# ltinphan/convex-mpc-unitree-go2

Measured on AMD Instinct MI355X. Metric: batched QP solves/sec (N=16, 4-leg friction cone) at 1/2/4/8 MI355X, higher is better.
Workload: dtype f32

## Files before the change

convex-mpc-unitree-go2_amd/csrc/cmpc_condense.h:

```cpp
#pragma once
#include "cmpc_instance.h"

namespace cmpc {

template <int NC>
__device__ __forceinline__ void condense_finish(Smem<NC>& s, f4 (&M)[Cfg<NC>::NTL], int n,
                                                float shift) {
  using C = Cfg<NC>;
  const int lane = opaque_lane();
  const int g = lane >> 4, c = lane & 15;
#pragma unroll
  for (int I = 0; I < C::TT; ++I) {
    const float rs = s.Rt[16 * I + c] + shift;
#pragma unroll
    for (int J = 0; J <= I; ++J) {
      if (J != I && 16 * I + 16 <= n) continue;
      f4 v = M[tile_index(I, J)];
      const int col = 16 * J + c;
#pragma unroll
      for (int q = 0; q < 4; ++q) {
        const int row = 16 * I + 4 * g + q;
        const bool pad = row >= n || col >= n;
        if (J == I) {
          const bool dg = 4 * g + q == c;
// ... 195 lines not shown
        if (kI[J] >= t) continue;
        f4 d = {0.f, 0.f, 0.f, 0.f};
#pragma unroll
        for (int q = 0; q < 3; ++q) d = mfma4(aA[q], Gd[J][q], d);
        Gd[J] = d;
      }
    }
    const int p0 = s.off[t], p1 = s.off[t + 1];
#pragma unroll
    for (int J = 0; J < C::TT; ++J) {
      if (16 * J + 15 < p0 || 16 * J >= p1) continue;
      const int p = 16 * J + c;
      if (p >= p0 && p < p1) {
        const float* bp = &s.Bt[p * kBS + 3 * g];
        Gd[J] = f4{bp[0], bp[1], bp[2], 0.f};
      }
    }
#pragma unroll
    for (int I = 0; I < C::TT; ++I) {
      if (16 * I + 15 < p0 || 16 * I >= p1) continue;
      const int p = 16 * I + c;
      float a[3] = {0.f, 0.f, 0.f};
      if (p >= p0 && p < p1) {
#pragma unroll
        for (int q = 0; q < 3; ++q) a[q] = Cs[p * 12 + 3 * g + q];
      }
#pragma unroll
      for (int J = 0; J <= I; ++J) {
        f4 acc = M[tile_index(I, J)];
#pragma unroll
        for (int q = 0; q < 3; ++q) acc = mfma4(a[q], Gd[J][q], acc);
        M[tile_index(I, J)] = acc;
      }
    }
  }
  mirror_diagonals<NC>(s, M, n, N);
  condense_finish<NC>(s, M, n, shift);
}

__device__ __forceinline__ void step_sums(int k, int N, float& S0, float& S1, float& S2) {
  S0 = (float)(N - k);
  S1 = (float)((N * (N - 1) - k * (k - 1)) >> 1);
  S2 = (float)(((N - 1) * N * (2 * N - 1) - (k - 1) * k * (2 * k - 1)) / 6);
}

template <int NC>
__device__ __forceinline__ void condense_tiles_nil(Smem<NC>& s, const KParams& P,
                                                   f4 (&M)[Cfg<NC>::NTL], int n, float shift) {
  using C = Cfg<NC>;
  const int lane = opaque_lane();
  const int g = lane >> 4, c = lane & 15;
  const int N = P.N;
  n = uniform(n);
  const int TA = (n + 15) >> 4;
  float* Vs = s.G;
  {
    const int sc = lane_state(c);
    float aN[3];
#pragma unroll
    for (int q = 0; q < 3; ++q) {
      const int r = 3 * g + q;
      aN[q] = (sc >= 0) ? s.A[sc * 12 + r] - ((sc == r) ? 1.f : 0.f) : 0.f;
    }
    WSYNC();
#pragma unroll
    for (int J = 0; J < C::TT; ++J) {
      if (J >= TA) continue;
      const int p = 16 * J + c;
      float bt[3];
#pragma unroll
      for (int q = 0; q < 3; ++q) bt[q] = (p < n) ? s.Bt[p * kBS + 3 * g + q] : 0.f;
      f4 d = {0.f, 0.f, 0.f, 0.f};
#pragma unroll
      for (int q = 0; q < 3; ++q) d = mfma4(aN[q], bt[q], d);
#pragma unroll
      for (int q = 0; q < 3; ++q) Vs[p * 12 + 3 * g + q] = d[q];
    }
  }
  WSYNC();
  float q2[3];
#pragma unroll
  for (int q = 0; q < 3; ++q) q2[q] = s.Q2[3 * g + q];
  float uc[C::TT][3], vc[C::TT][3];
#pragma unroll
  for (int J = 0; J < C::TT; ++J) {
    const int p = 16 * J + c;
    const bool ok = J < TA && p < n;
    const float kf = ok ? (float)s.par[p] : 0.f;
#pragma unroll
    for (int q = 0; q < 3; ++q) {
      vc[J][q] = ok ? Vs[p * 12 + 3 * g + q] : 0.f;
      uc[J][q] = ok ? fmaf(-kf, vc[J][q], s.Bt[p * kBS + 3 * g + q]) : 0.f;
    }
  }
#pragma unroll
  for (int I = 0; I < C::TT; ++I) {
    if (I >= TA) {
#pragma unroll
      for (int J = 0; J <= I; ++J) M[tile_index(I, J)] = f4{0.f, 0.f, 0.f, 0.f};
      continue;
    }
    float x[3], y[3];
    {
      const int p = 16 * I + c;
      const bool ok = p < n;
      const int k = ok ? s.par[p] : 0;
      float S0, S1, S2;
      step_sums(k, N, S0, S1, S2);
#pragma unroll
      for (int q = 0; q < 3; ++q) {
        const float v = vc[I][q];
        const float u = uc[I][q];
        x[q] = q2[q] * fmaf(S0, u, S1 * v);
        y[q] = q2[q] * fmaf(S1, u, S2 * v);
      }
    }
#pragma unroll
    for (int J = 0; J <= I; ++J) {
      float u[3], v[3];
#pragma unroll
      for (int q = 0; q < 3; ++q) {
        u[q] = uc[J][q];
        v[q] = vc[J][q];
      }
      f4 acc = {0.f, 0.f, 0.f, 0.f};
#pragma unroll
      for (int q = 0; q < 3; ++q) acc = mfma4(x[q], u[q], acc);
#pragma unroll
      for (int q = 0; q < 3; ++q) acc = mfma4(y[q], v[q], acc);
      M[tile_index(I, J)] = acc;
    }
  }
  mirror_diagonals<NC>(s, M, n, N);
  condense_finish<NC>(s, M, n, shift);
}

template <class SM>
__device__ __forceinline__ bool nilpotent_step(SM& s) {
  const int lane = opaque_lane();
  WSYNC();
  bool nz = false;
#pragma unroll
  for (int e0 = 0; e0 < 144; e0 += 64) {
    const int e = e0 + lane;
    if (e < 144) {
      const int i = e / 12, j = e % 12;
      float acc = 0.f;
#pragma unroll
      for (int k = 0; k < 12; ++k) {
        const float nik = s.A[i * 12 + k] - ((i == k) ? 1.f : 0.f);
        const float nkj = s.A[k * 12 + j] - ((k == j) ? 1.f : 0.f);
        acc = fmaf(nik, nkj, acc);
      }
      nz |= acc != 0.f;
    }
  }
  return __any(nz) == 0;
}

template <int NC>
__device__ __forceinline__ void condense_tiles(Smem<NC>& s, const KParams& P,
                                               f4 (&M)[Cfg<NC>::NTL], int n, float shift,
                                               bool nil = false) {
  if (nil) {
    condense_tiles_nil<NC>(s, P, M, n, shift);
    return;
  }
  if constexpr (NC <= 128) {
    if (P.latency_mode) {
      condense_tiles_bc<NC>(s, P, M, n, shift);
      return;
    }
  }
  condense_tiles_fwd<NC>(s, P, M, n, shift);
}

}
```

convex-mpc-unitree-go2_amd/csrc/cmpc_factor.h:

```cpp
#pragma once
#include "cmpc_instance.h"

namespace cmpc {

__device__ __forceinline__ float diag_element(const f4& d, int c) {
  const int qs = c & 3;
  return qs == 0 ? d[0] : qs == 1 ? d[1] : qs == 2 ? d[2] : d[3];
}

constexpr int kSweepPipeMaxNC = 128;
template <int NC, int K, class SM>
__device__ __forceinline__ void sweep_publish(SM& s, const f4 (&M)[Cfg<NC>::NTL], int sub,
                                              int g, int c) {
  using C = Cfg<NC>;
  const int c0 = 4 * sub;
  const int pc = c - c0;
  const bool colw = pc >= 0 && pc < 4;
  if (colw) {
#pragma unroll
    for (int I = K; I < C::TT; ++I) {
      f4 m = M[tile_index(I, K)];
      if (I == K) {
#pragma unroll
        for (int q = 0; q < 4; ++q) m[q] -= (4 * g + q == c) ? 1.f : 0.f;
// ... 128 lines not shown
        sweep_mfma<NC, -1, false, K>(M, a, b, TA);
        sweep_diagfix<NC, K>(M, sub, g, c);
      }
    }
    sweep_block_plain<NC, K + 1>(s, M, ng, TA, g, c);
  }
}

template <int NC, class SM>
__device__ __forceinline__ void ldl_tiles(SM& s, f4 (&M)[Cfg<NC>::NTL], int n) {
  using C = Cfg<NC>;
  const int lane = opaque_lane();
  const int g = lane >> 4, c = lane & 15;
  n = uniform(n);
  const int TA = (n + 15) >> 4;
#pragma unroll
  for (int I = 0; I < C::TT; ++I) {
    const float dg = diag_element(M[tile_index(I, I)], c);
    const int p = 16 * I + c;
    const float r = (p < n && dg > 0.f) ? rsqrtf(dg) : 1.f;
    if ((c >> 2) == g) s.ds[p] = r;
  }
  WSYNC();
#pragma unroll
  for (int I = 0; I < C::TT; ++I) {
    const f4 ri = *reinterpret_cast<const f4*>(&s.ds[16 * I + 4 * g]);
#pragma unroll
    for (int J = 0; J <= I; ++J) {
      const float cj = s.ds[16 * J + c];
      f4& m = M[tile_index(I, J)];
#pragma unroll
      for (int q = 0; q < 4; ++q) m[q] *= ri[q] * cj;
    }
  }
  const int ng = (n + 3) >> 2;
  if constexpr (NC <= kSweepPipeMaxNC) {
    if (ng > 0) {
      float a[C::TT], b[C::TT];
      sweep_publish<NC, 0>(s, M, 0, g, c);
      sweep_operands<NC, 0>(s, 0, g, c, a, b);
      sweep_block<NC, 0>(s, M, ng, TA, g, c, a, b);
    }
  } else {
    sweep_block_plain<NC, 0>(s, M, ng, TA, g, c);
  }
  float* rinvs = s.pan;
  WSYNC();
  const int lane_r = opaque_lane();
  const int g_r = lane_r >> 4, c_r = lane_r & 15;
#pragma unroll
  for (int p0 = 0; p0 < NC; p0 += 64) {
    const int p = p0 + lane_r;
    if (p < NC) rinvs[p] = 1.f / s.ds[p];
  }
  WSYNC();
#pragma unroll
  for (int I = 0; I < C::TT; ++I) {
    const f4 ri = *reinterpret_cast<const f4*>(&s.ds[16 * I + 4 * g_r]);
    const f4 rinv = *reinterpret_cast<const f4*>(&rinvs[16 * I + 4 * g_r]);
#pragma unroll
    for (int J = 0; J <= I; ++J) {
      const float cj = s.ds[16 * J + c_r];
      f4& m = M[tile_index(I, J)];
#pragma unroll
      for (int q = 0; q < 4; ++q) m[q] *= (J < I) ? rinv[q] * cj : -(ri[q] * cj);
    }
  }
}

template <int NC, class SM>
__device__ __forceinline__ void ldl_apply(SM& s, const f4 (&M)[Cfg<NC>::NTL], int n,
                                          const float* in, float* out) {
  using C = Cfg<NC>;
  CMPC_T0(t_sv);
  const int lane = opaque_lane();
  const int g = lane >> 4, c = lane & 15;
  n = uniform(n);
  const int TA = (n + 15) >> 4;
  WSYNC();
  float zc[C::TT];
  float bc[C::TT];
#pragma unroll
  for (int I = 0; I < C::TT; ++I) bc[I] = 0.f;
#pragma unroll
  for (int I = 0; I < C::TT; ++I) {
    if (I >= TA) {
      if (c == 0) *reinterpret_cast<f4*>(&out[16 * I + 4 * g]) = f4{0.f, 0.f, 0.f, 0.f};
      continue;
    }
    f4 zr = *reinterpret_cast<const f4*>(&in[16 * I + 4 * g]);
    if (I > 0) {
      f2 r01 = {0.f, 0.f}, r23 = {0.f, 0.f};
#pragma unroll
      for (int J = 0; J < I; ++J) {
        const f4 m = M[tile_index(I, J)];
        const f2 zj = {zc[J], zc[J]};
        r01 = __builtin_elementwise_fma(f2{m[0], m[1]}, zj, r01);
        r23 = __builtin_elementwise_fma(f2{m[2], m[3]}, zj, r23);
      }
      zr[0] -= row16_sum(r01[0]);
      zr[1] -= row16_sum(r01[1]);
      zr[2] -= row16_sum(r23[0]);
      zr[3] -= row16_sum(r23[1]);
    }
#pragma unroll
    for (int q = 0; q < 4; ++q) zr[q] = (16 * I + 4 * g + q < n) ? zr[q] : 0.f;
    if (c == 0) *reinterpret_cast<f4*>(&out[16 * I + 4 * g]) = zr;
    WSYNC();
    zc[I] = out[16 * I + c];
  }
#pragma unroll
  for (int I = C::TT - 1; I >= 0; --I) {
    if (I >= TA) continue;
    const f4 zr = *reinterpret_cast<const f4*>(&out[16 * I + 4 * g]);
    const f4 d = M[tile_index(I, I)];
    const float t =
        fmaf(d[3], zr[3], fmaf(d[2], zr[2], fmaf(d[1], zr[1], fmaf(d[0], zr[0], -bc[I]))));
    float xc = col4_sum(t);
    xc = (16 * I + c < n) ? xc : 0.f;
    WSYNC();
    if (g == 0) out[16 * I + c] = xc;
    if (I == 0) break;
    WSYNC();
    const f4 xr = *reinterpret_cast<const f4*>(&out[16 * I + 4 * g]);
#pragma unroll
    for (int J = 0; J < I; ++J) {
      const f4 m = M[tile_index(I, J)];
      bc[J] = fmaf(m[3], xr[3], fmaf(m[2], xr[2], fmaf(m[1], xr[1], fmaf(m[0], xr[0], bc[J]))));
    }
  }
  WSYNC();
  CMPC_ACC(3, t_sv);
  CMPC_CNT(13, 1);
}

template <int NC>
__device__ __forceinline__ void park_store(float* __restrict__ park, const f4 (&M)[Cfg<NC>::NTL]) {
  const int lane = opaque_lane();
#pragma unroll
  for (int t = 0; t < Cfg<NC>::NTL; ++t)
    *reinterpret_cast<f4*>(&park[t * 256 + lane * 4]) = M[t];
}

template <int NC>
__device__ __forceinline__ void park_load(const float* __restrict__ park, f4 (&M)[Cfg<NC>::NTL]) {
  const int lane = opaque_lane();
  asm volatile("s_waitcnt vmcnt(0)\n\tbuffer_inv sc1" ::: "memory");
#pragma unroll
  for (int t = 0; t < Cfg<NC>::NTL; ++t)
    M[t] = *reinterpret_cast<const f4*>(&park[t * 256 + lane * 4]);
}

}
```

convex-mpc-unitree-go2_amd/csrc/cmpc_gradient.h:

```cpp
#pragma once
#include "cmpc_condense.h"

namespace cmpc {

template <class SM>
__device__ __forceinline__ void gradient_powers(SM& s, f4 (&pw)[4], f4 (&tw)[4]) {
  const int lane = opaque_lane();
  const int g = lane >> 4, c = lane & 15;
  const int sc = lane_state(c);
  f4 Pd = {0.f, 0.f, 0.f, 0.f}, Td = {0.f, 0.f, 0.f, 0.f};
#pragma unroll
  for (int q = 0; q < 3; ++q) {
    const int r = 3 * g + q;
    Pd[q] = (sc >= 0) ? s.A[r * 12 + sc] : 0.f;
    Td[q] = (sc >= 0) ? s.A[sc * 12 + r] : 0.f;
  }
  pw[0] = Pd;
  tw[0] = Td;
  if (uniform(s.nil)) {
#pragma unroll
    for (int l = 1; l < 4; ++l) {
#pragma unroll
      for (int q = 0; q < 4; ++q) {
        const float dl = (sc == 3 * g + q && q < 3) ? 1.f : 0.f;
        pw[l][q] = fmaf((float)(1 << l), Pd[q] - dl, dl);
        tw[l][q] = fmaf((float)(1 << l), Td[q] - dl, dl);
      }
    }
    return;
  }
#pragma unroll
  for (int l = 1; l < 4; ++l) {
    f4 pn = {0.f, 0.f, 0.f, 0.f}, tn = {0.f, 0.f, 0.f, 0.f};
#pragma unroll
    for (int q = 0; q < 3; ++q) {
      pn = mfma4(tw[l - 1][q], pw[l - 1][q], pn);
      tn = mfma4(pw[l - 1][q], tw[l - 1][q], tn);
    }
    pw[l] = pn;
    tw[l] = tn;
  }
}

template <int NC, int W>
constexpr bool kGradLat = W > 1 || (Cfg<NC>::WPE == 1 && NC <= 160);
template <int NC, bool LAT = false, bool PREC = false>
__device__ __forceinline__ void gradient(Smem<NC>& s, const KParams& P, int n, const float* vin,
                                         float* gout, const f4* pwc = nullptr,
                                         const f4* twc = nullptr) {
  CMPC_T0(t_gr);
  const int lane = opaque_lane();
  const int g = lane >> 4, c = lane & 15;
  const int N = P.N;
  n = uniform(n);
  WSYNC();
  f4 Et = {0.f, 0.f, 0.f, 0.f};
  double Eh[3] = {0.0, 0.0, 0.0};
  if constexpr (LAT) {
    const int cc = (c < N) ? c : 0;
    const int p0 = s.off[cc], p1 = s.off[cc + 1];
    float dt[3], bv[12][3], vv[12];
#pragma unroll
    for (int q = 0; q < 3; ++q) dt[q] = s.Dt[12 * cc + 3 * g + q];
#pragma unroll
    for (int i = 0; i < 12; ++i) {
      const int p = min(p0 + i, NC - 1);
#pragma unroll
      for (int q = 0; q < 3; ++q) bv[i][q] = s.Bt[p * kBS + 3 * g + q];
      vv[i] = vin[p];
    }
    if constexpr (PREC) {
#pragma unroll
      for (int q = 0; q < 3; ++q) Eh[q] = (double)dt[q];
#pragma unroll
      for (int i = 0; i < 12; ++i) {
        const bool ok = p0 + i < p1;
#pragma unroll
        for (int q = 0; q < 3; ++q) Eh[q] = ok ? fma((double)bv[i][q], (double)vv[i], Eh[q]) : Eh[q];
      }
#pragma unroll
      for (int q = 0; q < 3; ++q) {
        if (c >= N) Eh[q] = 0.0;
        Et[q] = (float)Eh[q];
      }
    } else {
#pragma unroll
      for (int q = 0; q < 3; ++q) Et[q] = dt[q];
#pragma unroll
      for (int i = 0; i < 12; ++i) {
        const bool ok = p0 + i < p1;
#pragma unroll
        for (int q = 0; q < 3; ++q) Et[q] = ok ? fmaf(bv[i][q], vv[i], Et[q]) : Et[q];
      }
      if (c >= N) Et = f4{0.f, 0.f, 0.f, 0.f};
    }
  } else if (c < N) {
    const int p1 = s.off[c + 1];
    if constexpr (PREC) {
#pragma unroll
      for (int q = 0; q < 3; ++q) Eh[q] = (double)s.Dt[12 * c + 3 * g + q];
      for (int p = s.off[c]; p < p1; ++p) {
        const float* bt = &s.Bt[p * kBS + 3 * g];
        const double vp = (double)vin[p];
#pragma unroll
        for (int q = 0; q < 3; ++q) Eh[q] = fma((double)bt[q], vp, Eh[q]);
      }
#pragma unroll
      for (int q = 0; q < 3; ++q) Et[q] = (float)Eh[q];
    } else {
#pragma unroll
      for (int q = 0; q < 3; ++q) Et[q] = s.Dt[12 * c + 3 * g + q];
      for (int p = s.off[c]; p < p1; ++p) {
        const float* bt = &s.Bt[p * kBS + 3 * g];
        const float vp = vin[p];
#pragma unroll
        for (int q = 0; q < 3; ++q) Et[q] = fmaf(bt[q], vp, Et[q]);
      }
    }
  }
  if (uniform(s.nil)) {
    const int sc = lane_state(c);
    float aN[3], aNt[3];
#pragma unroll
    for (int q = 0; q < 3; ++q) {
      const int r = 3 * g + q;
      const float dl = (sc == r) ? 1.f : 0.f;
      aN[q] = (sc >= 0) ? s.A[sc * 12 + r] - dl : 0.f;
      aNt[q] = (sc >= 0) ? s.A[r * 12 + sc] - dl : 0.f;
    }
    if constexpr (PREC) {
      double u64[3];
#pragma unroll
      for (int q = 0; q < 3; ++q) {
        double x = Eh[q], y;
        row_scan2<false>(x, y);
        Eh[q] = x;
        u64[q] = y;
      }
      const int sr = ((c >> 2) < 3) ? 3 * (c & 3) + (c >> 2) : -1;
      d4 acc = {Eh[0], Eh[1], Eh[2], 0.0};
#pragma unroll
      for (int q = 0; q < 3; ++q) {
        const int r = 3 * g + q;
        const double a = (sr >= 0) ? (double)(s.A[sr * 12 + r] - ((sr == r) ? 1.f : 0.f)) : 0.0;
        acc = __builtin_amdgcn_mfma_f64_16x16x4f64(a, u64[q], acc, 0, 0, 0);
      }
#pragma unroll
      for (int q = 0; q < 3; ++q) Et[q] = (float)acc[q];
    } else {
    f4 u = {0.f, 0.f, 0.f, 0.f};
#pragma unroll
    for (int q = 0; q < 3; ++q) {
      float x = Et[q], y;
      row_scan2<false>(x, y);
      Et[q] = x;
      u[q] = y;
    }
#pragma unroll
    for (int q = 0; q < 3; ++q) Et = mfma4(aN[q], u[q], Et);
    }
    if (c < N) {
#pragma unroll
      for (int q = 0; q < 3; ++q) s.E[12 * c + 3 * g + q] = Et[q];
    }
    f4 Lt = {0.f, 0.f, 0.f, 0.f}, v = {0.f, 0.f, 0.f, 0.f};
#pragma unroll
    for (int q = 0; q < 3; ++q) {
      float x = (c < N) ? s.Q2[3 * g + q] * Et[q] : 0.f, y;
      row_scan2<true>(x, y);
      Lt[q] = x;
      v[q] = y;
    }
#pragma unroll
    for (int q = 0; q < 3; ++q) Lt = mfma4(aNt[q], v[q], Lt);
    if (c < N) {
#pragma unroll
      for (int q = 0; q < 3; ++q) s.L[12 * c + 3 * g + q] = Lt[q];
    }
  } else {
  f4 pw[4], tw[4];
  if (pwc != nullptr) {
#pragma unroll
    for (int l = 0; l < 4; ++l) {
      pw[l] = pwc[l];
      tw[l] = twc[l];
    }
  } else {
    gradient_powers(s, pw, tw);
  }
#pragma unroll
  for (int l = 0; l < 4; ++l) {
    if ((1 << l) >= N) break;
    f4 sh = {0.f, 0.f, 0.f, 0.f};
#pragma unroll
    for (int q = 0; q < 3; ++q) sh[q] = row_shift_pow2<false>(Et[q], l);
#pragma unroll
    for (int q = 0; q < 3; ++q) Et = mfma4(tw[l][q], sh[q], Et);
  }
  if (c < N) {
#pragma unroll
    for (int q = 0; q < 3; ++q) s.E[12 * c + 3 * g + q] = Et[q];
  }
  f4 Lt = {0.f, 0.f, 0.f, 0.f};
#pragma unroll
  for (int q = 0; q < 3; ++q) Lt[q] = (c < N) ? s.Q2[3 * g + q] * Et[q] : 0.f;
#pragma unroll
  for (int l = 0; l < 4; ++l) {
    if ((1 << l) >= N) break;
    f4 sh = {0.f, 0.f, 0.f, 0.f};
#pragma unroll
    for (int q = 0; q < 3; ++q) sh[q] = row_shift_pow2<true>(Lt[q], l);
#pragma unroll
    for (int q = 0; q < 3; ++q) Lt = mfma4(pw[l][q], sh[q], Lt);
  }
  if (c < N) {
#pragma unroll
    for (int q = 0; q < 3; ++q) s.L[12 * c + 3 * g + q] = Lt[q];
  }
  }
  WSYNC();
  for (int p = lane; p < n; p += 64) {
    const int k = s.par[p];
    const f4* l = reinterpret_cast<const f4*>(&s.L[12 * k]);
    f2 a2 = {s.Rt[p] * vin[p], 0.f};
    const f4* bt = reinterpret_cast<const f4*>(&s.Bt[p * kBS]);
#pragma unroll
    for (int j = 0; j < 3; ++j) {
      const f4 lv = l[j], bv = bt[j];
      a2 = __builtin_elementwise_fma(f2{bv[0], bv[1]}, f2{lv[0], lv[1]}, a2);
      a2 = __builtin_elementwise_fma(f2{bv[2], bv[3]}, f2{lv[2], lv[3]}, a2);
    }
    gout[p] = a2[0] + a2[1];
  }
  WSYNC();
  CMPC_ACC(2, t_gr);
  CMPC_CNT(12, 1);
}

}
```

convex-mpc-unitree-go2_amd/csrc/cmpc_solve.h:

```cpp
#pragma once
#include "cmpc_team.hip"

#include "cmpc_condense.h"
#include "cmpc_factor.h"
#include "cmpc_gradient.h"
#include "cmpc_polish.h"

namespace cmpc {

template <int NC>
__device__ __forceinline__ int session_start(Smem<NC>& s, const KParams& P, int ntri, int nfail,
                                             int& ntried, bool& seen) {
  const int l = opaque_lane();
  WSYNC();
  uint8_t c = 0;
  if (l < ntri) {
    c = (uint8_t)s.code[l];
    s.tpat[0][l] = c;
  }
  ntried = 1;
  seen = false;
#pragma unroll
  for (int k = 0; k < kFailMem; ++k) {
    if (k >= nfail) break;
    const bool diff = (l < ntri) && (s.fpat[k][l] != c);
    seen |= (__any(diff) == 0);
  }
  if (seen) return 0;
  return (nfail >= 2) ? min(P.polish_repairs, kLateRepairs) : P.polish_repairs;
}

template <int NC>
__device__ __forceinline__ bool tried_before(Smem<NC>& s, int ntri, int ntried) {
  const int l = opaque_lane();
  WSYNC();
  const uint8_t c = (l < ntri) ? (uint8_t)s.tcnt[l] : 0;
  bool hit = false;
  for (int k = 0; k < ntried; ++k) {
    const bool diff = (l < ntri) && (s.tpat[k][l] != c);
    hit |= (__any(diff) == 0);
  }
  return hit;
}


template <int NC>
constexpr bool kRhoLow = (NC == 128) || (kRhoLowHeavy && NC > 128);

struct Instance {
  int64_t b;
  int N, NP;
  Terrain T;
  bool weights_ok;
  float r2_min;
  const float* Bg;
  const float* xrb;
  int ntri, n;
  bool nil;
  const f4* pwc;
  const f4* twc;
};

struct Ctl {
  int status = -2, iters = 0;
  bool polished = false;
  float rp = 0.f, rd = 0.f, np_ = 0.f, nd = 0.f;
  float rho = 0.f;
  bool rho_low = false;
  int stable = 0;
  bool refactor = false;
  bool in_polish = false;
  int nact = 0;
  float shift = 0.f;
  int it = 0;
  int repairs_left = 0;
  int nadd = 0;
  bool from_cand = false;
  bool parked = false;
  int nfail = 0;
  int ntried = 0;
  bool seen_start = false;
  int last_pol = 0;
  bool fail_rho_done = false;
  bool warm_session = false;
};

__device__ __forceinline__ void set_rho(Ctl& c, const KParams& P, float rho, bool low) {
  c.rho = rho;
  c.rho_low = low;
  c.shift = uniformf(P.sigma + c.rho);
  c.refactor = true;
}

template <int NC>
__device__ __forceinline__ void stage_instance(Smem<NC>& s, const KParams& P, const Inputs& in,
                                               Instance& I, int lane) {
  const int64_t b = I.b;
  const int N = I.N, NP = I.NP;
  const Terrain T = I.T;
  bool weights_ok = true;
  float r2_min = P.r2_min;
  const float* Ab = in.Ad + b * 144;
  const float* Bg = in.Bd + b * (int64_t)N * 144;
  const float* gdb = in.gd + b * 12;
  const float* x0b = in.x0 + b * 12;
  const float* xrb = in.xref + b * (int64_t)N * 12;
  const uint8_t* ctb = in.contact + b * (int64_t)4 * N;

  WSYNC();
  const uint8_t ctv = (lane < 4 * N) ? ctb[(lane & 3) * N + (lane >> 2)] : (uint8_t)0;
  float bw[36];
  if (lane < 4 * N) {
    const float* src = Bg + lane * 36;
#pragma unroll
    for (int i = 0; i < 36; ++i) bw[i] = src[i];
  } else {
#pragma unroll
    for (int i = 0; i < 36; ++i) bw[i] = 0.f;
  }
  {
    float av[3], rv[4];
#pragma unroll
    for (int i = 0; i < 3; ++i) {
      const int e = lane + 64 * i;
      av[i] = (e < 144) ? Ab[e] : 0.f;
    }
#pragma unroll
    for (int i = 0; i < 4; ++i) {
      const int e = lane + 64 * i;
      rv[i] = (e < 12) ? x0b[e] : (e < 12 * (N + 1)) ? xrb[e - 12] : 0.f;
    }
    const float gv = (lane < 12) ? gdb[lane] : 0.f;
    if (in.Q || in.R) {
      const float q = (in.Q && lane < 12) ? in.Q[b * 12 + lane] : 0.f;
      const float r = (in.R && lane < 12) ? in.R[b * 12 + lane] : 1.f;
      weights_ok = __any(!(q >= 0.f && isfinite(q) && r > 0.f && isfinite(r))) == 0;
      if (lane < 12) {
        if (in.Q) s.Q2[lane] = weights_ok ? 2.f * q : 0.f;
        if (in.R) s.R2[lane] = weights_ok ? 2.f * r : 2.f;
      }
      if (in.R)
        r2_min = weights_ok ? uniformf(-wave_max((lane < 12) ? -2.f * r : -INFINITY)) : 2.f;
    }
#pragma unroll
    for (int i = 0; i < 3; ++i) {
      const int e = lane + 64 * i;
      if (e < 144) s.A[e] = av[i];
    }
#pragma unroll
    for (int i = 0; i < 4; ++i) s.G[lane + 64 * i] = rv[i];
    if (lane < 12) s.G[256 + lane] = gv;
  }
  const bool stc = lane < 4 * N && terrain_valid(T) && weights_ok && ctv != 0;
  const int pos = wave_excl_scan4(stc ? 1 : 0);
  const int ntri = wave_total4(stc ? 1 : 0);
  if (stc) s.tri[pos] = lane;
  if (lane < 4 * N) s.tri_of[lane] = stc ? pos : -1;
  WSYNC();
  {
    for (int o = lane; o < NP; o += 64) {
      const int k = o / 12, r = o % 12;
      const float* rk = &s.G[12 * k];
      float acc = s.G[256 + r] - rk[12 + r];
#pragma unroll
      for (int j = 0; j < 12; ++j) acc = fmaf(s.A[r * 12 + j], rk[j], acc);
      s.D[o] = acc;
    }
    build_admm_basis<NC>(s, P, Bg, ntri, &bw, __ballot(stc));
  }
  const bool nil = nilpotent_step(s);
  if (lane == 0) s.nil = nil ? 1 : 0;
// ... 281 lines not shown
    if (__any((nc & oc) != oc) == 0 && c.nadd + nf <= dd_max(NC)) {
      CMPC_T0(t_dd);
      dd = face_downdate<NC>(s, I.T, M, c.nact, ntri, c.nadd);
      TRACEF(I.b, "it %d downdate nf %d -> %d nadd %d\n", c.it, nf, (int)dd, c.nadd);
      CMPC_ACC(28, t_dd);
      CMPC_CNT(29, 1);
      CMPC_CNT(30, nf);
    }
  }
  if (lane < ntri) {
    s.code[lane] = s.tcnt[lane];
    if (c.ntried < kTryMem) s.tpat[c.ntried][lane] = (uint8_t)s.tcnt[lane];
  }
  if (c.ntried < kTryMem) ++c.ntried;
  if (dd) return;
  refactor_faces<NC>(s, P, I, c, s.z);
}

template <int NC>
__device__ __forceinline__ void warm_restart(Smem<NC>& s, const KParams& P, const Instance& I,
                                             Ctl& c) {
  c.warm_session = false;
  build_admm_basis<NC>(s, P, I.Bg, I.ntri);
  {
    const int l = opaque_lane();
    for (int p = l; p < I.n; p += 64) { s.x[p] = 0.f; s.z[p] = 0.f; s.y[p] = 0.f; }
    s.pcode[l] = -1;
  }
  WSYNC();
  c.in_polish = false;
  c.nact = I.n;
  c.nadd = 0;
  set_rho(c, P, kRhoLow<NC> ? 0.5f * P.rho0 : P.rho0, kRhoLow<NC>);
  c.stable = 0;
  c.last_pol = 0;
  c.ntried = 0;
  c.seen_start = false;
  c.parked = false;
}

template <int NC, int W>
__device__ __forceinline__ void session_failed(Smem<NC>& s, const KParams& P, const Instance& I,
                                               Ctl& c, f4 (&M)[TeamCfg<NC, W>::SLOTS],
                                               float* __restrict__ park, TeamSmem<NC, W>* ts,
                                               int* seq, Diag& diag, int lane) {
  c.warm_session = false;
  TRACEF(I.b, "it %d SESSION-FAIL nfail %d seen %d parked %d rho_low %d fail_rho_done %d nadd %d\n",
         c.it, c.nfail, (int)c.seen_start, (int)c.parked, (int)c.rho_low, (int)c.fail_rho_done,
         c.nadd);
  diag.session_failed();
  if (!c.seen_start) {
    const int l = opaque_lane();
    if (l < I.ntri) s.fpat[c.nfail % kFailMem][l] = s.tpat[0][l];
    ++c.nfail;
  }
  build_admm_basis<NC>(s, P, I.Bg, I.ntri);
  c.in_polish = false;
  c.nact = I.n;
  if (c.nfail == 1 && !c.seen_start && kFailRho != 1.f && !c.fail_rho_done) {
    c.fail_rho_done = true;
    set_rho(c, P, uniformf(kFailRho * P.rho0), false);
    return;
  }
  if (c.rho_low) {
    set_rho(c, P, uniformf(P.rho0), false);
    return;
  }
  c.shift = uniformf(P.sigma + c.rho);
  if (c.parked) {
    restore_tiles<NC, W>(park, ts, seq, M);
  } else {
    c.refactor = true;
  }
}

template <int NC, int W>
__device__ __forceinline__ bool admm_iteration(Smem<NC>& s, const KParams& P, const Instance& I,
                                               Ctl& c, const f4 (&M)[TeamCfg<NC, W>::SLOTS],
                                               TeamSmem<NC, W>* ts, int* seq, int lane) {
  const int n = I.n, ntri = I.ntri, it = c.it;
  const Terrain T = I.T;
  const float alpha = P.alpha;
  float rho = c.rho;
  gradient<NC, kGradLat<NC, W>>(s, P, n, s.x, s.g, I.pwc, I.twc);
  {
    const int l = opaque_lane();
    if (l < ntri) {
#pragma unroll
      for (int a = 0; a < 3; ++a) {
        const int p = 3 * l + a;
        s.r[p] = rho * (s.z[p] - s.x[p]) - s.g[p] - s.y[p];
      }
    }
  }
  apply_factors<NC, W>(s, ts, seq, M, n, s.r, s.dl);
  CMPC_T0(t_rest);
  const bool last = (it == P.max_iter);
  const bool adapt = P.adaptive_interval > 0 && (it % P.adaptive_interval) == 0;
  const float inv_rho = 1.f / rho;
  float lrp = 0.f, lrd = 0.f, lnp = 0.f, lnd = 0.f;
  bool changed = false;
  {
    const int l = opaque_lane();
    if (l < ntri) {
      float w[3], xr[3], xs[3];
#pragma unroll
      for (int a = 0; a < 3; ++a) {
        const int p = 3 * l + a;
        const float x = s.x[p], z = s.z[p];
        const float xt = x + s.dl[p];
        xr[a] = alpha * xt + (1.f - alpha) * z;
        xs[a] = alpha * xt + (1.f - alpha) * x;
        w[a] = xr[a] + s.y[p] * inv_rho;
      }
      float pv[3];
      const int code = project(w[0], w[1], w[2], T.mu, T.fz_min, pv[0], pv[1], pv[2]);
#pragma unroll
      for (int a = 0; a < 3; ++a) {
        const int p = 3 * l + a;
        const float zn = pv[a];
        const float yn = s.y[p] + rho * (xr[a] - zn);
        s.x[p] = xs[a];
        s.z[p] = zn;
        s.y[p] = yn;
        const float gp = s.g[p];
        lrp = fmaxf(lrp, fabsf(xs[a] - zn));
        lrd = fmaxf(lrd, fabsf(gp + yn));
        lnp = fmaxf(lnp, fmaxf(fabsf(xs[a]), fabsf(zn)));
        lnd = fmaxf(lnd, fmaxf(fabsf(gp), fabsf(yn)));
      }
      changed = code != s.pcode[l];
      s.pcode[l] = code;
      s.code[l] = code;
    }
  }
  if (trace_on(I.b)) {
    const float trp = wave_max(lrp), trd = wave_max(lrd);
    TRACEF(I.b, "it %d rho %g rp %g rd %g stable %d\n", it, rho, trp, trd, c.stable);
  }
  c.stable = (__any(changed) != 0) ? 0 : c.stable + 1;
  bool do_pol = false;
  const int pstable = P.polish_stable;
  const int backoff = pstable << min(c.nfail, kBackoffCap);
  int need = pstable;
  for (int f = 0; f < min(c.nfail, kBackoffCap); ++f) need *= kStableGrow;
  if (c.stable >= need && !last && it - c.last_pol >= backoff &&
      (P.check_every == 1 || it % P.check_every == 0)) {
    do_pol = true;
    c.last_pol = it;
    c.stable = -backoff;
  }
  if (adapt || last) {
    c.rp = wave_max(lrp); c.rd = wave_max(lrd); c.np_ = wave_max(lnp); c.nd = wave_max(lnd);
  }
  if (adapt && !last) {
    float q = rho * sqrtf((c.rp / fmaxf(c.np_, 1e-30f)) / (c.rd / fmaxf(c.nd, 1e-30f) + 1e-30f));
    q = fminf(fmaxf(q, 1e-6f), 1e6f);
    if (q > 5.f * rho || q < 0.2f * rho) set_rho(c, P, uniformf(q), false);
  }
  CMPC_ACC(7, t_rest);
  return do_pol;
}

template <int NC, int W>
__device__ __forceinline__ void start_session(Smem<NC>& s, const KParams& P, const Instance& I,
                                              Ctl& c, const f4 (&M)[TeamCfg<NC, W>::SLOTS],
                                              float* __restrict__ park, TeamSmem<NC, W>* ts,
                                              int* seq, Diag& diag, int lane) {
  CMPC_CNT(9, 1);
  diag.polish_attempt();
  CMPC_T0(t_ps);
  const bool pending = c.refactor;
  c.parked = !c.refactor && !c.rho_low && c.nfail > 0;
  if (c.parked) park_tiles<NC, W>(park, ts, seq, M);
  enter_polish<NC>(s, P, I, c);
  TRACEF(I.b, "it %d SESSION nfail %d parked %d rho %g refactor_pending %d seen %d repairs %d nact %d\n",
         c.it, c.nfail, (int)c.parked, c.rho, (int)pending, (int)c.seen_start, c.repairs_left,
         c.nact);
  CMPC_ACC(14, t_ps);
}

template <int NC>
__device__ __forceinline__ int force_triple(const Smem<NC>& s, int o, int& a) {
  const int k = o / 12, l = (o % 12) / 3;
  a = o % 3;
  return s.tri_of[4 * k + l];
}

template <int NC>
__device__ __forceinline__ bool write_w(Smem<NC>& s, const Instance& I, float* wb, bool polished,
                                        int lane) {
  const int NP = I.NP;
  const float* uf = polished ? s.x : s.z;
  int bad = 0;
  for (int o = lane; o < NP; o += 64) {
    const float xv = s.E[o] + I.xrb[o];
    int a;
    const int t = force_triple(s, o, a);
    const float uv = (t >= 0) ? uf[3 * t + a] : 0.f;
    bad |= !(isfinite(xv) && isfinite(uv));
    wb[o] = xv;
    wb[NP + o] = uv;
  }
  return __any(bad) == 0;
}

template <int NC, int W>
__device__ __forceinline__ void write_y(Smem<NC>& s, const KParams& P, const Instance& I,
                                        float* yb, bool polished, int lane) {
  const int NP = I.NP;
  if (polished && I.n > 0) {
    build_admm_basis<NC>(s, P, I.Bg, I.ntri);
    gradient<NC, kGradLat<NC, W>>(s, P, I.n, s.x, s.g, I.pwc, I.twc);
  }
  const float* yf = polished ? s.g : s.y;
  const float sg = polished ? -1.f : 1.f;
  for (int o = lane; o < NP; o += 64) {
    int a;
    const int t = force_triple(s, o, a);
    yb[o] = (t >= 0) ? sg * yf[3 * t + a] : 0.f;
  }
}

template <int NC>
__device__ __forceinline__ void write_lam(Smem<NC>& s, const Instance& I, float* lb, bool polished,
                                          int lane) {
  const int N = I.N, NP = I.NP;
  const Terrain T = I.T;
  if (!I.weights_ok) {
    for (int o = lane; o < 52 * N; o += 64) lb[o] = 0.f;
// ... 150 lines not shown
```

convex-mpc-unitree-go2_amd/csrc/cmpc_wave_prims.h:

```cpp
#pragma once
#include <hip/hip_runtime.h>
#include <stdint.h>

namespace cmpc {

typedef float f4 __attribute__((ext_vector_type(4)));
typedef float f2 __attribute__((ext_vector_type(2)));

__device__ __forceinline__ float readlane_f(float v, int lane) {
  return __int_as_float(__builtin_amdgcn_readlane(__float_as_int(v), lane));
}

template <int CTRL>
__device__ __forceinline__ float dpp(float v) {
  return __int_as_float(__builtin_amdgcn_mov_dpp(__float_as_int(v), CTRL, 0xF, 0xF, true));
}

__device__ __forceinline__ int uniform(int v) { return __builtin_amdgcn_readfirstlane(v); }
__device__ __forceinline__ float uniformf(float v) {
  return __builtin_bit_cast(float, __builtin_amdgcn_readfirstlane(__builtin_bit_cast(int, v)));
}

__device__ __forceinline__ void pair32(float v, float& a, float& b) {
  const auto r = __builtin_amdgcn_permlane32_swap(__float_as_int(v), __float_as_int(v), false, false);
  a = __int_as_float(r[0]);
  b = __int_as_float(r[1]);
}
__device__ __forceinline__ void pair16(float v, float& a, float& b) {
  const auto r = __builtin_amdgcn_permlane16_swap(__float_as_int(v), __float_as_int(v), false, false);
  a = __int_as_float(r[0]);
  b = __int_as_float(r[1]);
}

__device__ __forceinline__ float wave_max(float v) {
  v = fmaxf(v, dpp<0xB1>(v));
  v = fmaxf(v, dpp<0x4E>(v));
  v = fmaxf(v, dpp<0x141>(v));
  v = fmaxf(v, dpp<0x140>(v));
  float a, b;
  pair32(v, a, b);
  v = fmaxf(a, b);
  pair16(v, a, b);
  return fmaxf(a, b);
}

__device__ __forceinline__ int wave_excl_scan4(int v) {
  const unsigned long long b0 = __ballot(v & 1), b1 = __ballot(v & 2);
  const int c0 = __builtin_amdgcn_mbcnt_hi((unsigned)(b0 >> 32), __builtin_amdgcn_mbcnt_lo((unsigned)b0, 0));
  const int c1 = __builtin_amdgcn_mbcnt_hi((unsigned)(b1 >> 32), __builtin_amdgcn_mbcnt_lo((unsigned)b1, 0));
  return c0 + 2 * c1;
}
__device__ __forceinline__ int wave_total4(int v) {
  return __popcll(__ballot(v & 1)) + 2 * __popcll(__ballot(v & 2));
}

__device__ __forceinline__ f4 mfma4(float a, float b, f4 c) {
  return __builtin_amdgcn_mfma_f32_16x16x4f32(a, b, c, 0, 0, 0);
}

typedef double d4 __attribute__((ext_vector_type(4)));

template <int CTRL>
__device__ __forceinline__ double dpp64(double v) {
  const long long b = __double_as_longlong(v);
  const int lo = __builtin_amdgcn_mov_dpp((int)(unsigned)(b & 0xffffffffll), CTRL, 0xF, 0xF, true);
  const int hi = __builtin_amdgcn_mov_dpp((int)(b >> 32), CTRL, 0xF, 0xF, true);
  return __longlong_as_double(((long long)hi << 32) | (long long)(unsigned)lo);
}

__device__ __forceinline__ float row16_sum(float v) {
  v += dpp<0xB1>(v);
  v += dpp<0x4E>(v);
  v += dpp<0x141>(v);
  v += dpp<0x140>(v);
  return v;
}

template <bool SHL, int D>
__device__ __forceinline__ float row_shift(float v) { return dpp<(SHL ? 0x100 : 0x110) + D>(v); }
template <bool SHL, int D>
__device__ __forceinline__ double row_shift(double v) { return dpp64<(SHL ? 0x100 : 0x110) + D>(v); }
template <bool SHL>
__device__ __forceinline__ float row_shift_pow2(float v, int l) {
  switch (l) {
    case 0: return row_shift<SHL, 1>(v);
    case 1: return row_shift<SHL, 2>(v);
    case 2: return row_shift<SHL, 4>(v);
    default: return row_shift<SHL, 8>(v);
  }
}
template <bool SHL, class T>
__device__ __forceinline__ void row_scan2(T& x, T& y) {
  x += row_shift<SHL, 1>(x);
  x += row_shift<SHL, 2>(x);
  x += row_shift<SHL, 4>(x);
  x += row_shift<SHL, 8>(x);
  y = row_shift<SHL, 1>(x);
  y += row_shift<SHL, 1>(y);
  y += row_shift<SHL, 2>(y);
  y += row_shift<SHL, 4>(y);
  y += row_shift<SHL, 8>(y);
}

__device__ __forceinline__ float col4_sum(float v) {
  float a, b;
  pair32(v, a, b);
  pair16(a + b, a, b);
  return a + b;
}

__device__ __forceinline__ float wave_sum(float v) { return col4_sum(row16_sum(v)); }

__device__ __forceinline__ int opaque_lane() {
  int l = threadIdx.x & 63;
  asm volatile("" : "+v"(l));
  return l;
}

#define WSYNC() asm volatile("" ::: "memory")

#include "cmpc_diag.h"
#ifdef CMPC_STAMPS
__device__ unsigned long long g_stamps[32];
#define CMPC_FENCE()                                            \
  do {                                                          \
    __builtin_amdgcn_sched_barrier(0);                          \
    asm volatile("s_waitcnt vmcnt(0) lgkmcnt(0)" ::: "memory"); \
    __builtin_amdgcn_sched_barrier(0);                          \
  } while (0)
#define CMPC_T0(name) \
  CMPC_FENCE();       \
  const unsigned long long name = __builtin_amdgcn_s_memtime()
#define CMPC_ACC(ph, t0)                                                              \
  do {                                                                                \
    CMPC_FENCE();                                                                     \
    const unsigned long long _t1 = __builtin_amdgcn_s_memtime();                      \
    if (threadIdx.x == 0) s.st[ph] += _t1 - (t0);                                     \
  } while (0)
#define CMPC_CNT(ph, v) \
  do { if (threadIdx.x == 0) s.st[ph] += (unsigned long long)(v); } while (0)
#else
#define CMPC_T0(name) (void)0
#define CMPC_ACC(ph, t0) (void)0
#define CMPC_CNT(ph, v) (void)0
#endif

}
```

Baseline: 9.474 million.

## Fuse ADMM rhs into gradient epilogue and pipeline triangular solve reductions

Bundles several micro-optimizations: the ADMM right-hand side is now computed inside the gradient close loop through an epilogue lambda, which removes a separate pass over shared memory. The forward LDL substitution is software-pipelined, accumulating the next tile's off-diagonal products early, and its four row reductions are interleaved. Padding masks are precomputed per lane and the backward loads are prefetched. DPP scans are interleaved across the three components, parent indices are cached in registers, and integer modulo is replaced by counters and a cached 1/rho. These cut dependency chains and ALU work per ADMM iteration, at the cost of more register pressure and some added code complexity.

```diff
diff --git a/convex-mpc-unitree-go2_amd/csrc/cmpc_condense.h b/convex-mpc-unitree-go2_amd/csrc/cmpc_condense.h
--- a/convex-mpc-unitree-go2_amd/csrc/cmpc_condense.h
+++ b/convex-mpc-unitree-go2_amd/csrc/cmpc_condense.h
@@ -301,11 +301,13 @@
 #pragma unroll
   for (int q = 0; q < 3; ++q) q2[q] = s.Q2[3 * g + q];
   float uc[C::TT][3], vc[C::TT][3];
+  int kc[C::TT];
 #pragma unroll
   for (int J = 0; J < C::TT; ++J) {
     const int p = 16 * J + c;
     const bool ok = J < TA && p < n;
-    const float kf = ok ? (float)s.par[p] : 0.f;
+    kc[J] = ok ? s.par[p] : 0;
+    const float kf = (float)kc[J];
 #pragma unroll
     for (int q = 0; q < 3; ++q) {
       vc[J][q] = ok ? Vs[p * 12 + 3 * g + q] : 0.f;
@@ -321,11 +323,8 @@
     }
     float x[3], y[3];
     {
-      const int p = 16 * I + c;
-      const bool ok = p < n;
-      const int k = ok ? s.par[p] : 0;
       float S0, S1, S2;
-      step_sums(k, N, S0, S1, S2);
+      step_sums(kc[I], N, S0, S1, S2);
 #pragma unroll
       for (int q = 0; q < 3; ++q) {
         const float v = vc[I][q];
diff --git a/convex-mpc-unitree-go2_amd/csrc/cmpc_factor.h b/convex-mpc-unitree-go2_amd/csrc/cmpc_factor.h
--- a/convex-mpc-unitree-go2_amd/csrc/cmpc_factor.h
+++ b/convex-mpc-unitree-go2_amd/csrc/cmpc_factor.h
@@ -234,47 +234,64 @@
   float bc[C::TT];
 #pragma unroll
   for (int I = 0; I < C::TT; ++I) bc[I] = 0.f;
+  if (4 * lane < NC) *reinterpret_cast<f4*>(&out[4 * lane]) = f4{0.f, 0.f, 0.f, 0.f};
+  const int nl = n - 16 * (TA - 1);
+  const bool kr0 = 4 * g < nl, kr1 = 4 * g + 1 < nl, kr2 = 4 * g + 2 < nl, kr3 = 4 * g + 3 < nl;
+  const bool kc = c < nl;
+  f2 a01 = {0.f, 0.f}, a23 = {0.f, 0.f};
 #pragma unroll
   for (int I = 0; I < C::TT; ++I) {
-    if (I >= TA) {
-      if (c == 0) *reinterpret_cast<f4*>(&out[16 * I + 4 * g]) = f4{0.f, 0.f, 0.f, 0.f};
-      continue;
-    }
+    if (I >= TA) continue;
     f4 zr = *reinterpret_cast<const f4*>(&in[16 * I + 4 * g]);
+    f2 n01 = {0.f, 0.f}, n23 = {0.f, 0.f};
     if (I > 0) {
-      f2 r01 = {0.f, 0.f}, r23 = {0.f, 0.f};
-#pragma unroll
-      for (int J = 0; J < I; ++J) {
-        const f4 m = M[tile_index(I, J)];
-        const f2 zj = {zc[J], zc[J]};
-        r01 = __builtin_elementwise_fma(f2{m[0], m[1]}, zj, r01);
-        r23 = __builtin_elementwise_fma(f2{m[2], m[3]}, zj, r23);
-      }
-      zr[0] -= row16_sum(r01[0]);
-      zr[1] -= row16_sum(r01[1]);
-      zr[2] -= row16_sum(r23[0]);
-      zr[3] -= row16_sum(r23[1]);
-    }
-#pragma unroll
-    for (int q = 0; q < 4; ++q) zr[q] = (16 * I + 4 * g + q < n) ? zr[q] : 0.f;
+      const f4 ml = M[tile_index(I, I - 1)];
+      const f2 zl = {zc[I - 1], zc[I - 1]};
+      const f2 r01 = __builtin_elementwise_fma(f2{ml[0], ml[1]}, zl, a01);
+      const f2 r23 = __builtin_elementwise_fma(f2{ml[2], ml[3]}, zl, a23);
+      if (I + 1 < C::TT) {
+#pragma unroll
+        for (int J = 0; J < I; ++J) {
+          const f4 m = M[tile_index(I + 1, J)];
+          const f2 zj = {zc[J], zc[J]};
+          n01 = __builtin_elementwise_fma(f2{m[0], m[1]}, zj, n01);
+          n23 = __builtin_elementwise_fma(f2{m[2], m[3]}, zj, n23);
+        }
+      }
+      float s0 = r01[0], s1 = r01[1], s2 = r23[0], s3 = r23[1];
+      row16_sum4(s0, s1, s2, s3);
+      zr[0] -= s0;
+      zr[1] -= s1;
+      zr[2] -= s2;
+      zr[3] -= s3;
+    }
+    a01 = n01;
+    a23 = n23;
+    const bool whole = I < TA - 1;
+    zr[0] = (whole | kr0) ? zr[0] : 0.f;
+    zr[1] = (whole | kr1) ? zr[1] : 0.f;
+    zr[2] = (whole | kr2) ? zr[2] : 0.f;
+    zr[3] = (whole | kr3) ? zr[3] : 0.f;
     if (c == 0) *reinterpret_cast<f4*>(&out[16 * I + 4 * g]) = zr;
     WSYNC();
     zc[I] = out[16 * I + c];
   }
+  f4 zr = {0.f, 0.f, 0.f, 0.f};
+  if (TA > 0) zr = *reinterpret_cast<const f4*>(&out[16 * (TA - 1) + 4 * g]);
 #pragma unroll
   for (int I = C::TT - 1; I >= 0; --I) {
     if (I >= TA) continue;
-    const f4 zr = *reinterpret_cast<const f4*>(&out[16 * I + 4 * g]);
     const f4 d = M[tile_index(I, I)];
     const float t =
         fmaf(d[3], zr[3], fmaf(d[2], zr[2], fmaf(d[1], zr[1], fmaf(d[0], zr[0], -bc[I]))));
     float xc = col4_sum(t);
-    xc = (16 * I + c < n) ? xc : 0.f;
+    xc = ((I < TA - 1) | kc) ? xc : 0.f;
     WSYNC();
     if (g == 0) out[16 * I + c] = xc;
     if (I == 0) break;
     WSYNC();
     const f4 xr = *reinterpret_cast<const f4*>(&out[16 * I + 4 * g]);
+    zr = *reinterpret_cast<const f4*>(&out[16 * (I - 1) + 4 * g]);
 #pragma unroll
     for (int J = 0; J < I; ++J) {
       const f4 m = M[tile_index(I, J)];
diff --git a/convex-mpc-unitree-go2_amd/csrc/cmpc_gradient.h b/convex-mpc-unitree-go2_amd/csrc/cmpc_gradient.h
--- a/convex-mpc-unitree-go2_amd/csrc/cmpc_gradient.h
+++ b/convex-mpc-unitree-go2_amd/csrc/cmpc_gradient.h
@@ -44,10 +44,15 @@
 
 template <int NC, int W>
 constexpr bool kGradLat = W > 1 || (Cfg<NC>::WPE == 1 && NC <= 160);
-template <int NC, bool LAT = false, bool PREC = false>
+template <int NC>
+constexpr bool kCloseUnrolled = NC <= 160;
+struct NoEpilogue {
+  __device__ __forceinline__ void operator()(int, float, bool) const {}
+};
+template <int NC, bool LAT = false, bool PREC = false, class EPI = NoEpilogue>
 __device__ __forceinline__ void gradient(Smem<NC>& s, const KParams& P, int n, const float* vin,
                                          float* gout, const f4* pwc = nullptr,
-                                         const f4* twc = nullptr) {
+                                         const f4* twc = nullptr, EPI epi = EPI()) {
   CMPC_T0(t_gr);
   const int lane = opaque_lane();
   const int g = lane >> 4, c = lane & 15;
@@ -130,13 +135,7 @@
     }
     if constexpr (PREC) {
       double u64[3];
-#pragma unroll
-      for (int q = 0; q < 3; ++q) {
-        double x = Eh[q], y;
-        row_scan2<false>(x, y);
-        Eh[q] = x;
-        u64[q] = y;
-      }
+      row_scan2x3<false>(Eh, u64);
       const int sr = ((c >> 2) < 3) ? 3 * (c & 3) + (c >> 2) : -1;
       d4 acc = {Eh[0], Eh[1], Eh[2], 0.0};
 #pragma unroll
@@ -148,14 +147,10 @@
 #pragma unroll
       for (int q = 0; q < 3; ++q) Et[q] = (float)acc[q];
     } else {
-    f4 u = {0.f, 0.f, 0.f, 0.f};
-#pragma unroll
-    for (int q = 0; q < 3; ++q) {
-      float x = Et[q], y;
-      row_scan2<false>(x, y);
-      Et[q] = x;
-      u[q] = y;
-    }
+    float S[3] = {Et[0], Et[1], Et[2]}, u[3];
+    row_scan2x3<false>(S, u);
+#pragma unroll
+    for (int q = 0; q < 3; ++q) Et[q] = S[q];
 #pragma unroll
     for (int q = 0; q < 3; ++q) Et = mfma4(aN[q], u[q], Et);
     }
@@ -163,14 +158,11 @@
 #pragma unroll
       for (int q = 0; q < 3; ++q) s.E[12 * c + 3 * g + q] = Et[q];
     }
-    f4 Lt = {0.f, 0.f, 0.f, 0.f}, v = {0.f, 0.f, 0.f, 0.f};
-#pragma unroll
-    for (int q = 0; q < 3; ++q) {
-      float x = (c < N) ? s.Q2[3 * g + q] * Et[q] : 0.f, y;
-      row_scan2<true>(x, y);
-      Lt[q] = x;
-      v[q] = y;
-    }
+    float Rs[3], v[3];
+#pragma unroll
+    for (int q = 0; q < 3; ++q) Rs[q] = (c < N) ? s.Q2[3 * g + q] * Et[q] : 0.f;
+    row_scan2x3<true>(Rs, v);
+    f4 Lt = {Rs[0], Rs[1], Rs[2], 0.f};
 #pragma unroll
     for (int q = 0; q < 3; ++q) Lt = mfma4(aNt[q], v[q], Lt);
     if (c < N) {
@@ -219,8 +211,10 @@
   }
   }
   WSYNC();
-  for (int p = lane; p < n; p += 64) {
-    const int k = s.par[p];
+  auto close_trip = [&](int p0) {
+    const bool ok = p0 + lane < n;
+    const int p = ok ? p0 + lane : 0;
+    const int k = ok ? s.par[p] : 0;
     const f4* l = reinterpret_cast<const f4*>(&s.L[12 * k]);
     f2 a2 = {s.Rt[p] * vin[p], 0.f};
     const f4* bt = reinterpret_cast<const f4*>(&s.Bt[p * kBS]);
@@ -230,7 +224,15 @@
       a2 = __builtin_elementwise_fma(f2{bv[0], bv[1]}, f2{lv[0], lv[1]}, a2);
       a2 = __builtin_elementwise_fma(f2{bv[2], bv[3]}, f2{lv[2], lv[3]}, a2);
     }
-    gout[p] = a2[0] + a2[1];
+    const float gv = a2[0] + a2[1];
+    if (ok) gout[p] = gv;
+    epi(p, gv, ok);
+  };
+  if constexpr (kCloseUnrolled<NC>) {
+#pragma unroll
+    for (int p0 = 0; p0 < NC; p0 += 64) close_trip(p0);
+  } else {
+    for (int p0 = 0; p0 < n; p0 += 64) close_trip(p0);
   }
   WSYNC();
   CMPC_ACC(2, t_gr);
diff --git a/convex-mpc-unitree-go2_amd/csrc/cmpc_solve.h b/convex-mpc-unitree-go2_amd/csrc/cmpc_solve.h
--- a/convex-mpc-unitree-go2_amd/csrc/cmpc_solve.h
+++ b/convex-mpc-unitree-go2_amd/csrc/cmpc_solve.h
@@ -66,6 +66,7 @@
   bool polished = false;
   float rp = 0.f, rd = 0.f, np_ = 0.f, nd = 0.f;
   float rho = 0.f;
+  float inv_rho = 0.f;
   bool rho_low = false;
   int stable = 0;
   bool refactor = false;
@@ -73,6 +74,8 @@
   int nact = 0;
   float shift = 0.f;
   int it = 0;
+  int it_adapt = 0;
+  int it_check = 0;
   int repairs_left = 0;
   int nadd = 0;
   bool from_cand = false;
@@ -87,6 +90,7 @@
 
 __device__ __forceinline__ void set_rho(Ctl& c, const KParams& P, float rho, bool low) {
   c.rho = rho;
+  c.inv_rho = uniformf(1.f / rho);
   c.rho_low = low;
   c.shift = uniformf(P.sigma + c.rho);
   c.refactor = true;
@@ -534,22 +538,18 @@
   const Terrain T = I.T;
   const float alpha = P.alpha;
   float rho = c.rho;
-  gradient<NC, kGradLat<NC, W>>(s, P, n, s.x, s.g, I.pwc, I.twc);
-  {
-    const int l = opaque_lane();
-    if (l < ntri) {
-#pragma unroll
-      for (int a = 0; a < 3; ++a) {
-        const int p = 3 * l + a;
-        s.r[p] = rho * (s.z[p] - s.x[p]) - s.g[p] - s.y[p];
-      }
-    }
-  }
+  auto rhs = [&s, rho](int p, float gv, bool ok) {
+    const float rp = rho * (s.z[p] - s.x[p]) - gv - s.y[p];
+    if (ok) s.r[p] = rp;
+  };
+  gradient<NC, kGradLat<NC, W>, false, decltype(rhs)>(s, P, n, s.x, s.g, I.pwc, I.twc, rhs);
   apply_factors<NC, W>(s, ts, seq, M, n, s.r, s.dl);
   CMPC_T0(t_rest);
   const bool last = (it == P.max_iter);
-  const bool adapt = P.adaptive_interval > 0 && (it % P.adaptive_interval) == 0;
-  const float inv_rho = 1.f / rho;
+  if (++c.it_adapt == P.adaptive_interval) c.it_adapt = 0;
+  if (++c.it_check == P.check_every) c.it_check = 0;
+  const bool adapt = P.adaptive_interval > 0 && c.it_adapt == 0;
+  const float inv_rho = c.inv_rho;
   float lrp = 0.f, lrd = 0.f, lnp = 0.f, lnd = 0.f;
   bool changed = false;
   {
@@ -597,7 +597,7 @@
   int need = pstable;
   for (int f = 0; f < min(c.nfail, kBackoffCap); ++f) need *= kStableGrow;
   if (c.stable >= need && !last && it - c.last_pol >= backoff &&
-      (P.check_every == 1 || it % P.check_every == 0)) {
+      (P.check_every == 1 || c.it_check == 0)) {
     do_pol = true;
     c.last_pol = it;
     c.stable = -backoff;
diff --git a/convex-mpc-unitree-go2_amd/csrc/cmpc_wave_prims.h b/convex-mpc-unitree-go2_amd/csrc/cmpc_wave_prims.h
--- a/convex-mpc-unitree-go2_amd/csrc/cmpc_wave_prims.h
+++ b/convex-mpc-unitree-go2_amd/csrc/cmpc_wave_prims.h
@@ -76,6 +76,13 @@
   return v;
 }
 
+__device__ __forceinline__ void row16_sum4(float& a, float& b, float& c, float& d) {
+  a += dpp<0xB1>(a), b += dpp<0xB1>(b), c += dpp<0xB1>(c), d += dpp<0xB1>(d);
+  a += dpp<0x4E>(a), b += dpp<0x4E>(b), c += dpp<0x4E>(c), d += dpp<0x4E>(d);
+  a += dpp<0x141>(a), b += dpp<0x141>(b), c += dpp<0x141>(c), d += dpp<0x141>(d);
+  a += dpp<0x140>(a), b += dpp<0x140>(b), c += dpp<0x140>(c), d += dpp<0x140>(d);
+}
+
 template <bool SHL, int D>
 __device__ __forceinline__ float row_shift(float v) { return dpp<(SHL ? 0x100 : 0x110) + D>(v); }
 template <bool SHL, int D>
@@ -100,6 +107,23 @@
   y += row_shift<SHL, 2>(y);
   y += row_shift<SHL, 4>(y);
   y += row_shift<SHL, 8>(y);
+}
+
+template <bool SHL, class T>
+__device__ __forceinline__ void row_scan2x3(T (&x)[3], T (&y)[3]) {
+#define CMPC_SCAN_STEP(v, D)   \
+  _Pragma("unroll") for (int q = 0; q < 3; ++q) v[q] += row_shift<SHL, D>(v[q])
+  CMPC_SCAN_STEP(x, 1);
+  CMPC_SCAN_STEP(x, 2);
+  CMPC_SCAN_STEP(x, 4);
+  CMPC_SCAN_STEP(x, 8);
+#pragma unroll
+  for (int q = 0; q < 3; ++q) y[q] = row_shift<SHL, 1>(x[q]);
+  CMPC_SCAN_STEP(y, 1);
+  CMPC_SCAN_STEP(y, 2);
+  CMPC_SCAN_STEP(y, 4);
+  CMPC_SCAN_STEP(y, 8);
+#undef CMPC_SCAN_STEP
 }
 
 __device__ __forceinline__ float col4_sum(float v) {
```

Result: faster. 9.875 million, median of 6 (+4.2%).
